# trucndt/oversim

Measured on AMD Instinct MI355X. Metric: routed lookup hops/sec (whole node), higher is better.
Workload: dtype u32 (160-bit keys), int64 ns, fp64 coordinates; 1 GPU; C: Chord 2^20 nodes per GPU (ring sharded over GPUs), 10M random-key iterative one-way lookups per GPU; overlay=chord, nodes_total=1048576, lookups_per_gpu=10000000, hopCountMax=50, parallelism=1 GPU, seed=0xc, successorListSize=8, routingType=iterative

## Files before the change

oversim_amd/csrc/chord.hip:

```cpp
#include <hipcub/hipcub.hpp>

#include "engine.hpp"
#include "launch.hpp"
#include "persist.hpp"

#include <algorithm>
#include <cstdio>
#include <vector>

namespace ovs {


__global__ void k_check_sorted(const KeyRec* __restrict__ recs, uint32_t n, uint32_t* bad)
{
    const uint32_t i = blockIdx.x * blockDim.x + threadIdx.x;
    if (i + 1 < n) {
        const K160 a = key_of(load_rec(recs, i)), b = key_of(load_rec(recs, i + 1));
        if (!k_lt(a, b)) atomicOr(bad, 1u);
    }
}

__global__ void k_chord_rowlen(const KeyRec* __restrict__ recs, uint32_t n, uint32_t lo, uint32_t cnt, uint64_t* rowlen)
{
    const uint32_t t = blockIdx.x * blockDim.x + threadIdx.x;
// ... 35 lines not shown
    FingerEnt* row = fingers + r.aux;
    for (int i = KEYBITS - 1; i >= ilo; --i)
        row[KEYBITS - 1 - i].idx = ring_lower_bound(recs, n, k_add(self, k_pow2(i)));
}

__global__ void k_chord_top(const KeyRec* __restrict__ recs, uint32_t n, int L, FingerEnt* __restrict__ ftop)
{
    const uint64_t t = (uint64_t)blockIdx.x * blockDim.x + threadIdx.x;
    if (t >= (uint64_t)n * (uint32_t)L) return;
    const uint32_t v = (uint32_t)(t / (uint32_t)L);
    const int i = KEYBITS - 1 - (int)(t % (uint32_t)L);
    const K160 self = key_of(load_rec(recs, v));
    ftop[t].idx = ring_lower_bound(recs, n, k_add(self, k_pow2(i)));
}

__global__ void k_chord_nodes(const KeyRec* __restrict__ recs, const double2* __restrict__ xy, uint32_t n, int ns,
                              NodeRec* __restrict__ nodes)
{
    const uint32_t v = blockIdx.x * blockDim.x + threadIdx.x;
    if (v >= n) return;
    const KeyRec r = load_rec(recs, v);
    const K160 C = key_of(r);
    const K160 P = key_of(load_rec(recs, v == 0 ? n - 1 : v - 1));
    const K160 S0 = key_of(load_rec(recs, v + 1 == n ? 0 : v + 1));
    const uint32_t sl = v + (uint32_t)ns >= n ? v + (uint32_t)ns - n : v + (uint32_t)ns;
    const K160 SL = key_of(load_rec(recs, sl));
    const double2 p = xy[v];
    const uint64_t gP = top64(k_sub(P, C)), gS0 = top64(k_sub(S0, C)), gSL = top64(k_sub(SL, C));
    uint4* o = reinterpret_cast<uint4*>(nodes + v);
    o[0] = make_uint4(r.w[0], r.w[1], r.w[2], r.w[3]);
    o[1] = make_uint4(r.w[4], r.aux, (uint32_t)__double2loint(p.x), (uint32_t)__double2hiint(p.x));
    o[2] = make_uint4((uint32_t)__double2loint(p.y), (uint32_t)__double2hiint(p.y), (uint32_t)gS0, (uint32_t)(gS0 >> 32));
    o[3] = make_uint4((uint32_t)gSL, (uint32_t)(gSL >> 32), (uint32_t)gP, (uint32_t)(gP >> 32));
}

__global__ void k_chord_win(const KeyRec* __restrict__ recs, uint32_t n, uint32_t lo, uint32_t cnt, int ns,
                            WinRec* __restrict__ win)
{
    const uint32_t t = blockIdx.x * blockDim.x + threadIdx.x;
    if (t >= cnt) return;
    const uint32_t v = lo + t;
    const K160 C = key_of(load_rec(recs, v));
    uint64_t g[8];
    for (int j = 0; j < 8; ++j) {
        uint32_t sj = v + (uint32_t)j + 1;
        while (sj >= n) sj -= n;
        g[j] = j < ns ? top64(k_sub(key_of(load_rec(recs, sj)), C)) : ~0ull;
    }
    uint4* o = reinterpret_cast<uint4*>(win + t);
    for (int j = 0; j < 4; ++j)
        o[j] = make_uint4((uint32_t)g[2 * j], (uint32_t)(g[2 * j] >> 32), (uint32_t)g[2 * j + 1], (uint32_t)(g[2 * j + 1] >> 32));
}

__global__ void k_chord_entries(const NodeRec* __restrict__ nodes, FingerEnt* __restrict__ ents, uint64_t total)
{
    const uint64_t e = (uint64_t)blockIdx.x * blockDim.x + threadIdx.x;
    if (e >= total) return;
    const uint32_t f = ents[e].idx;
    const uint4* q = reinterpret_cast<const uint4*>(nodes + f);
    const uint4 a = q[0], b = q[1], c = q[2], d = q[3];
    uint4* o = reinterpret_cast<uint4*>(ents + e);
    o[0] = a;
    o[1] = make_uint4(b.x, f, b.z, b.w);
    o[2] = c;
    o[3] = make_uint4(d.x, d.y, b.y, 0u);
}

__global__ void k_chord_export(const KeyRec* __restrict__ recs, const FingerEnt* __restrict__ fingers,
                               uint32_t n, uint32_t* __restrict__ out)
{
    const uint64_t t = (uint64_t)blockIdx.x * blockDim.x + threadIdx.x;
    if (t >= (uint64_t)n * KEYBITS) return;
    const uint32_t v = (uint32_t)(t / KEYBITS);
    const int pos = (int)(t % KEYBITS);
    const KeyRec r = load_rec(recs, v);
    const uint32_t s0i = v + 1 == n ? 0 : v + 1;
    const int ilo = k_msb(k_sub(key_of(load_rec(recs, s0i)), key_of(r))) + 1;
    out[t] = pos >= ilo ? fingers[r.aux + (KEYBITS - 1 - pos)].idx : s0i;
}


struct Decision {
    uint32_t next;
    KeyRec rec;
    uint8_t sib;
    uint8_t broken;
};

__device__ __forceinline__ uint32_t ring_next(uint32_t i, uint32_t d, uint32_t n)
{
    uint32_t j = i + d;
    return j >= n ? j - n : j;
}

__device__ __forceinline__ bool sibling_general(const ChordView& V, uint32_t self, const K160& K,
                                                int numSiblings)
{
    const uint32_t pred = V.pred[self];
    const int ssize = V.nsucc[self];
    const K160 C = key_of(load_rec(V.recs, self));
    if (pred == NONE) {
        const bool isEmpty = ssize == 0 || (ssize == 1 && V.succ[(uint64_t)self * V.sls] == self);
        return isEmpty || k_eq(C, K);
    }
    const K160 PK = key_of(load_rec(V.recs, pred));
    if (between_R(K, PK, C)) return true;
    (void)numSiblings;
    return false;
}

__device__ __forceinline__ Decision decide_general(const ChordView& V, uint32_t c, const KeyRec& crec,
                                                   const K160& K)
{
    Decision d;
    d.broken = 0; d.sib = 0;
    const K160 C = key_of(crec);
    const uint64_t sb = (uint64_t)c * V.sls;
    const int ssize = V.nsucc[c];
// ... 165 lines not shown
    }
}


__device__ __forceinline__ int shard_owner(const uint64_t* __restrict__ lo, int nsh, uint32_t c)
{
    int r = 0;
    for (int i = 1; i < nsh; ++i) r += ((uint64_t)c >= lo[i]) ? 1 : 0;
    return r;
}

__device__ __forceinline__ ovs_lookup_rec load_lrec(const ovs_lookup_rec* __restrict__ p, uint64_t i)
{
    const uint4* q = reinterpret_cast<const uint4*>(p + i);
    const uint4 a = q[0], b = q[1], c = q[2];
    ovs_lookup_rec r;
    r.key[0] = a.x; r.key[1] = a.y; r.key[2] = a.z; r.key[3] = a.w; r.key[4] = b.x;
    r.src = b.y; r.cur = b.z; r.qid = b.w;
    r.t_ns = (int64_t)((uint64_t)c.x | ((uint64_t)c.y << 32));
    r.hops = (uint16_t)(c.z & 0xFFFF);
    r.local = (uint8_t)((c.z >> 16) & 0xFF);
    return r;
}

__device__ __forceinline__ void store_lrec(ovs_lookup_rec* __restrict__ p, uint64_t i, const K160& K, uint32_t S,
                                           uint32_t cur, uint32_t qid, int64_t t, int hops, int local)
{
    uint4* q = reinterpret_cast<uint4*>(p + i);
    q[0] = make_uint4(K.w[0], K.w[1], K.w[2], K.w[3]);
    q[1] = make_uint4(K.w[4], S, cur, qid);
    q[2] = make_uint4((uint32_t)(uint64_t)t, (uint32_t)((uint64_t)t >> 32), (uint32_t)hops | ((uint32_t)local << 16), 0u);
}

enum : uint32_t { PH_FETCH = 0, PH_START = 1, PH_NODE = 2, PH_PROBE = 3, PH_WIN = 4 };

struct Hdr {
    K160 k;
    uint32_t row;
    double x, y;
    uint64_t gS0, gSL;
};

__device__ __forceinline__ void lds_wave_fence()
{
    __builtin_amdgcn_fence(__ATOMIC_RELEASE, "wavefront");
    __builtin_amdgcn_wave_barrier();
    __builtin_amdgcn_fence(__ATOMIC_ACQUIRE, "wavefront");
}

__device__ __forceinline__ int msb64(uint64_t x) { return 63 - __clzll((long long)x); }

__device__ __forceinline__ uint64_t u64(uint32_t lo, uint32_t hi) { return (uint64_t)lo | ((uint64_t)hi << 32); }

__device__ __forceinline__ int cmp_gap(const ChordView& V, const K160& D, uint64_t gt, const K160& C, uint32_t g)
{
    const uint64_t Dt = top64(D);
    if (Dt != gt) return Dt < gt ? -1 : 1;
    const K160 G = k_sub(key_of(load_rec(V.recs, g)), C);
    return k_lt(D, G) ? -1 : (k_eq(D, G) ? 0 : 1);
}

__device__ __forceinline__ uint64_t top64_sub(const K160& a, const K160& b)
{
    const bool borrow = (a.w[2] < b.w[2]) | ((a.w[2] == b.w[2]) & (lo64(a) < lo64(b)));
    return top64(a) - top64(b) - (borrow ? 1u : 0u);
}

struct LaneIO {
    const K160* __restrict__ qkeys;
    const uint32_t* __restrict__ qsrc;
    ovs_route_out* __restrict__ out;
    uint32_t* __restrict__ hopseq;
    const uint32_t* __restrict__ perm;
    const ovs_lookup_rec* __restrict__ in;
    const K160* __restrict__ fkeys;
    const uint32_t* __restrict__ fsrc;
    uint32_t fqid;
    ovs_lookup_rec* __restrict__ sout;
    uint64_t scap;
    unsigned long long* scount;
    ovs_done_rec* __restrict__ done;
    uint64_t dcap;
    unsigned long long* dcount;
    const uint64_t* __restrict__ shard_lo;
    int nsh, me;
    uint64_t n, chunk;
    ovs_lookup_rec* __restrict__ stage_hand;
    ovs_done_rec* __restrict__ stage_done;
    uint8_t* __restrict__ stag;
    unsigned long long* dyn;
    uint64_t dyn_from;
};

constexpr PersistTune K1_TUNE{0.70, 64};

#ifdef OVS_K1_TAIL
__device__ unsigned long long g_k1_tail[2 * PERSIST_TAIL_MAX];
#endif
#ifdef OVS_CHORD_STATS
__device__ unsigned long long g_k1_stats[8];
#endif

#ifndef OVS_K1_WAVES
#define OVS_K1_WAVES 5
#endif
#ifndef OVS_K1_SHARD_WAVES
#define OVS_K1_SHARD_WAVES 5
#endif
template <bool REC, bool RECORD, bool SHARD, bool LKC = false, bool DEF = false>
// ... 312 lines not shown
                cur = nx;
                if (via_node) {
                    nsib = nx_sib; pend = REC;
                    lp = reinterpret_cast<const uint4*>(V.nodes + nx);
                    ph = PH_NODE;
                    return false;
                }
                if (REC) t += DC.msgRoute + coord_ns(sx, sy, A.x, A.y, DC.round);
                asib = nx_sib;
                return true;
            };
            if (!fin && nxt != NONE) arrived = send(nxt, nxt_node, nxt_sib);

            if (arrived) {
                uint32_t nx2 = NONE;
                bool nx2_sib = false;
                const K160 D = k_sub(K, A.k);
                if (ph == PH_START) asib = k_zero(D) || cmp_gap(V, D, u64(L3.z, L3.w), A.k, cur == 0 ? V.n - 1 : cur - 1) > 0;
                if (SHARD && redo) {
                    redo = false;
                    local = false;
                    if (REC) { sx = A.x; sy = A.y; }
                } else if (REC) {
                    const bool at_src = local;
                    local = false;
                    sx = A.x; sy = A.y;
                    if (asib && (!at_src || hops < hcm)) { fin = true; R = cur; }
                    else if (asib || hops >= hcm) { fin = true; status = OVS_LOOKUP_HOPMAX; }
                } else if (local) {
                    local = false;
                    if (asib) { fin = true; R = S; }
                } else {
                    const int64_t cdr = coord_ns(sx, sy, A.x, A.y, DC.round);
                    if (!SHARD) cd = cdr;
                    const int64_t rtt = DC.msgCall + ((LKC && asib) ? DC.msgRespSib : DC.msgResp1) + 2 * cdr;
                    if (rtt >= DC.rpcTimeout) {
                        fin = true;
                        status = (t + DC.rpcTimeout > DC.lookupTimeout) ? OVS_LOOKUP_TIMEOUT : OVS_LOOKUP_RPC_TIMEOUT;
                    } else {
                        t += rtt;
                        if (t > DC.lookupTimeout) { fin = true; status = OVS_LOOKUP_TIMEOUT; }
                        else {
                            if (RECORD && !SHARD && hops < hcm) io.hopseq[dst * (uint64_t)hcm + hops] = cur;
                            ++hops;
                            if (asib) { fin = true; R = cur; }
                        }
                    }
                }
                if (!REC && !fin && hcm && hops >= hcm) { fin = true; status = OVS_LOOKUP_HOPMAX; }
                if (!fin) {
                    C = A.k; row = A.row; gSL = A.gSL; gTx = false;
                    if (!SHARD) Dt = top64(D);
                    const uint32_t s0 = ring_next(cur, 1, V.n);
                    if (cmp_gap(V, D, A.gS0, C, s0) <= 0) {
                        nx2 = s0; nx2_sib = true;
                    } else {
                        ilo = A.gS0 ? 97 + msb64(A.gS0) : k_msb(k_sub(key_of(load_rec(V.recs, s0)), C)) + 1;
                        esl = gSL ? 97 + msb64(gSL) : 96;
                        const uint32_t sl = ring_next(cur, (uint32_t)ns, V.n);
                        const int c = cmp_gap(V, D, gSL, C, sl);
                        if (c < 0) {
                            if (SHARD && remote) {
                                redo_hand();
                            } else {
                                lp = reinterpret_cast<const uint4*>(V.win + (cur - V.lo));
                                ph = PH_WIN;
                            }
                        } else {
                            gTx = c == 0;
                            fb = gTx ? ring_next(cur, (uint32_t)ns - 1, V.n) : sl;
                            pi = k_msb(D);
                            if (pi >= ilo) {
                                if (SHARD && remote && pi < KEYBITS - V.ftl) {
                                    redo_hand();
                                } else {
                                    lp = fptr(pi);
                                    ph = PH_PROBE;
                                }
                            } else {
                                nx2 = fb;
                            }
                        }
                    }
                }
                if (!fin && nx2 != NONE) send(nx2, true, nx2_sib);
            }

            if (fin) {
                ovs_route_out o;
                if (REC) {
                    const bool ok = status == OVS_LOOKUP_OK;
                    o.hops = (uint16_t)(ok ? hops : 0);
                    o.one_way_hops = (uint8_t)(ok ? hops : 0);
                    o.latency_ns = ok ? t : -1;
                    o.responsible = ok ? R : NONE;
                } else if (status == OVS_LOOKUP_OK) {
                    o.hops = (uint16_t)hops;
                    o.responsible = R;
                    o.one_way_hops = (uint8_t)(hops + (R != S ? 1 : 0));
                    o.latency_ns = t + ((R != S && !LKC) ? DC.msgRoute + (SHARD ? coord_ns(sx, sy, A.x, A.y, DC.round) : cd) : 0);
                } else {
                    o.hops = (uint16_t)hops;
                    o.responsible = NONE;
                    o.one_way_hops = 0;
                    o.latency_ns = -1;
                }
                o.status = status;
                if (SHARD) {
                    ovs_done_rec dr;
                    dr.qid = qid; dr.pad = 0; dr.out = o;
                    io.stage_done[q] = dr;
                    io.stag[q] = (uint8_t)io.nsh;
                } else {
                    static_assert(sizeof(ovs_route_out) == 16 && alignof(ovs_route_out) == 8, "one 16 B record");
                    reinterpret_cast<uint4*>(io.out)[dst] =
                        make_uint4(o.responsible, (uint32_t)o.hops | ((uint32_t)o.status << 16) | ((uint32_t)o.one_way_hops << 24),
                                   (uint32_t)(uint64_t)o.latency_ns, (uint32_t)((uint64_t)o.latency_ns >> 32));
// ... 103 lines not shown
    out[i] = 2 * bw + DC.access2 + coord_ns(p.x, p.y, r.x, r.y, DC.round);
}


hipError_t launch_check_sorted(const KeyRec* recs, uint32_t n, uint32_t* bad, hipStream_t s)
{
    if (n < 2) return hipSuccess;
    hipLaunchKernelGGL(k_check_sorted, dim3(nblk(n, 256)), dim3(256), 0, s, recs, n, bad);
    return hipGetLastError();
}

hipError_t launch_chord_build(KeyRec* recs, uint32_t n, uint32_t lo, uint32_t hi, FingerEnt** fingers_out,
                              uint64_t* nfing_out, hipStream_t s)
{
    hipError_t e;
    uint64_t* rowlen = nullptr;
    uint64_t* off = nullptr;
    void* tmp = nullptr;
    size_t tmpb = 0;
    const uint32_t cnt = hi - lo;
    *fingers_out = nullptr;
    if ((e = hipMalloc(&rowlen, sizeof(uint64_t) * (cnt + 1))) != hipSuccess) return e;
    if ((e = hipMalloc(&off, sizeof(uint64_t) * (cnt + 1))) != hipSuccess) { hipFree(rowlen); return e; }
    hipLaunchKernelGGL(k_chord_rowlen, dim3(nblk(cnt, 256)), dim3(256), 0, s, recs, n, lo, cnt, rowlen);
    hipMemsetAsync(rowlen + cnt, 0, sizeof(uint64_t), s);
    hipcub::DeviceScan::ExclusiveSum(nullptr, tmpb, rowlen, off, cnt + 1, s);
    if ((e = hipMalloc(&tmp, tmpb)) != hipSuccess) { hipFree(rowlen); hipFree(off); return e; }
    hipcub::DeviceScan::ExclusiveSum(tmp, tmpb, rowlen, off, cnt + 1, s);
    uint64_t total = 0;
    hipMemcpyAsync(&total, off + cnt, sizeof(uint64_t), hipMemcpyDeviceToHost, s);
    hipStreamSynchronize(s);
    if (total + KEYBITS >= 0xFFFFFFFFull) { hipFree(rowlen); hipFree(off); hipFree(tmp); return hipErrorInvalidValue; }
    FingerEnt* fing = nullptr;
    if ((e = hipMalloc(&fing, sizeof(FingerEnt) * (total + KEYBITS))) != hipSuccess) {
        hipFree(rowlen); hipFree(off); hipFree(tmp); return e;
    }
    hipMemsetAsync(fing, 0, sizeof(FingerEnt) * (total + KEYBITS), s);
    hipLaunchKernelGGL(k_set_aux, dim3(nblk(cnt, 256)), dim3(256), 0, s, recs, off, lo, cnt);
    hipLaunchKernelGGL(k_chord_fill, dim3(nblk(cnt, 128)), dim3(128), 0, s, recs, n, lo, cnt, fing);
    e = hipStreamSynchronize(s);
    hipFree(rowlen); hipFree(off); hipFree(tmp);
    if (e != hipSuccess) { hipFree(fing); return e; }
    *fingers_out = fing;
    *nfing_out = total;
    return hipGetLastError();
}

hipError_t launch_chord_nodes(const KeyRec* recs, const double2* xy, uint32_t n, int ns, NodeRec* nodes,
                              FingerEnt* fingers, uint64_t nfing, WinRec* win, uint32_t lo, uint32_t hi, hipStream_t s)
{
    if (n == 0) return hipSuccess;
    hipLaunchKernelGGL(k_chord_nodes, dim3(nblk(n, 256)), dim3(256), 0, s, recs, xy, n, ns, nodes);
    if (hi > lo) hipLaunchKernelGGL(k_chord_win, dim3(nblk(hi - lo, 256)), dim3(256), 0, s, recs, n, lo, hi - lo, ns, win);
    if (nfing) hipLaunchKernelGGL(k_chord_entries, dim3(nblk(nfing, 256)), dim3(256), 0, s, nodes, fingers, nfing);
    return hipGetLastError();
}

hipError_t launch_chord_top(const KeyRec* recs, uint32_t n, int L, FingerEnt* ftop, hipStream_t s)
{
    const uint64_t tot = (uint64_t)n * (uint32_t)L;
    if (tot == 0) return hipSuccess;
    hipLaunchKernelGGL(k_chord_top, dim3(nblk(tot, 256)), dim3(256), 0, s, recs, n, L, ftop);
    return hipGetLastError();
}

hipError_t launch_chord_entries(const NodeRec* nodes, FingerEnt* ents, uint64_t total, hipStream_t s)
{
    if (total == 0) return hipSuccess;
    hipLaunchKernelGGL(k_chord_entries, dim3(nblk(total, 256)), dim3(256), 0, s, nodes, ents, total);
    return hipGetLastError();
}

hipError_t launch_chord_export(const KeyRec* recs, const FingerEnt* fingers, uint32_t n, uint32_t* out,
                               hipStream_t s)
{
    const uint64_t tot = (uint64_t)n * KEYBITS;
    hipLaunchKernelGGL(k_chord_export, dim3(nblk(tot, 256)), dim3(256), 0, s, recs, fingers, n, out);
    return hipGetLastError();
}

template <bool REC, bool RECORD, bool SHARD, bool LKC = false, bool DEF = false>
static hipError_t lanes_launch(const ChordView& V, const DelayConsts& DC, const LookupConsts& LC, LaneIO io,
                               int num_cu, hipStream_t s)
{
    const PersistPlan pl = persist_plan(io.n, persist_waves<k_chord_lanes<REC, RECORD, SHARD, LKC, DEF>>(num_cu),
                                        io.dyn != nullptr, K1_TUNE);
    const uint64_t blocks = pl.blocks;
    io.chunk = pl.chunk;
    io.dyn_from = pl.dyn_from;
    if (!pl.dyn) io.dyn = nullptr;
#ifdef OVS_CHORD_STATS
    unsigned long long z[8] = {};
    hipMemcpyToSymbolAsync(HIP_SYMBOL(g_k1_stats), z, sizeof z, 0, hipMemcpyHostToDevice, s);
#endif
    hipLaunchKernelGGL((k_chord_lanes<REC, RECORD, SHARD, LKC, DEF>), dim3((unsigned)blocks), dim3(256), 0, s, V, DC,
                       LC, io);
#ifdef OVS_K1_TAIL
    if (!SHARD) persist_tail_report("k1tail", HIP_SYMBOL(g_k1_tail), blocks * 4, io.chunk, s);
#endif
#ifdef OVS_CHORD_STATS
    hipMemcpyFromSymbolAsync(z, HIP_SYMBOL(g_k1_stats), sizeof z, 0, hipMemcpyDeviceToHost, s);
    hipStreamSynchronize(s);
    fprintf(stderr, "k1stats n=%llu fetch=%llu start=%llu node=%llu probe1=%llu reprobe=%llu win=%llu "
            "wave_iters=%llu busy_lanes=%llu\n",
            (unsigned long long)io.n, z[0], z[1], z[2], z[3], z[4], z[5], z[6], z[7]);
#endif
    return hipGetLastError();
}

template <bool IDEAL, bool RECORD, bool REC>
static hipError_t chord_route_launch(const ChordView& V, const DelayConsts& DC, const LookupConsts& LC,
                                     const K160* qkeys, const uint32_t* qsrc, uint64_t nq, ovs_route_out* out,
                                     uint32_t* hopseq, int num_cu, hipStream_t s, const uint32_t* perm = nullptr,
                                     unsigned long long* dyn = nullptr)
{
    if constexpr (IDEAL) {
        LaneIO io{};
        io.qkeys = qkeys; io.qsrc = qsrc; io.out = out; io.hopseq = hopseq; io.n = nq; io.perm = perm;
        io.dyn = dyn;
        if constexpr (!REC && !RECORD) {
            if (DC.lookupCall) return lanes_launch<false, false, false, true>(V, DC, LC, io, num_cu, s);
        }
// ... 270 lines not shown
```

oversim_amd/csrc/engine.hpp:

```cpp
#pragma once
#include <hip/hip_runtime.h>
#include <stdint.h>

#include "key160.hpp"
#include "../../include/ovs_kbr.h"

namespace ovs {

constexpr uint32_t NONE = 0xFFFFFFFFu;
constexpr int KEYBITS = 160;

inline uint64_t up256(uint64_t b) { return (b + 255) & ~255ull; }

inline unsigned nblk(uint64_t n, unsigned b) { return (unsigned)((n + b - 1) / b); }

struct DelayConsts {
    int64_t msgCall;
    int64_t msgResp1;
    int64_t msgRoute;
    int64_t rpcTimeout;
    int64_t lookupTimeout;
    int32_t round;
    int32_t respBase;
    int32_t respPerNode;
    int32_t callBytes;
    int32_t routeBytes;
    double datarate;
    int64_t access2;
    int64_t msgRespSib;
    int32_t lookupCall;
    int64_t bwCall;
    int64_t bwRoute;
    int64_t bwResp[17];
};


__device__ __forceinline__ int64_t simtime_ns(double seconds, int round)
{
    const double x = __dmul_rn(seconds, 1e9);
    return round ? (int64_t)floor(__dadd_rn(x, 0.5)) : (int64_t)x;
}

__device__ __forceinline__ int64_t coord_ns(double ax, double ay, double bx, double by, int round)
{
    const double dx = __dsub_rn(ax, bx);
    const double dy = __dsub_rn(ay, by);
    const double s = __dadd_rn(__dmul_rn(dx, dx), __dmul_rn(dy, dy));
    const float f = __double2float_rn(__dsqrt_rn(s));
    return simtime_ns(__dmul_rn(0.001, (double)f), round);
}

__device__ __forceinline__ int64_t bw_ns(int32_t bytes, double datarate, int round)
{
    return simtime_ns(__ddiv_rn((double)((int64_t)bytes * 8), datarate), round);
// ... 1 lines not shown

__device__ __forceinline__ int64_t resp_ns(const DelayConsts& DC, int nodes)
{
    return 2 * bw_ns(DC.respBase + DC.respPerNode * nodes, DC.datarate, DC.round) + DC.access2;
}

__device__ __forceinline__ KeyRec load_rec(const KeyRec* __restrict__ recs, uint32_t i)
{
    const uint2* p = reinterpret_cast<const uint2*>(recs + i);
    const uint2 a = p[0], b = p[1], c = p[2];
    KeyRec r;
    r.w[0] = a.x; r.w[1] = a.y; r.w[2] = b.x; r.w[3] = b.y; r.w[4] = c.x; r.aux = c.y;
    return r;
}

__device__ __forceinline__ K160 rkey(const KeyRec* __restrict__ recs, uint64_t i) { return key_of(load_rec(recs + i, 0)); }

__device__ __forceinline__ uint64_t vis_bit(uint32_t x) { return 1ull << ((x * 0x9E3779B1u) >> 26); }

__device__ __forceinline__ ovs_route_out iter_route_out(uint8_t status, int hops, int64_t t, uint32_t responsible, uint32_t S,
                                                        double sx, double sy, double rx, double ry, const DelayConsts& DC)
{
    ovs_route_out o;
    o.hops = (uint16_t)hops;
    o.status = status;
    if (status == OVS_LOOKUP_OK) {
        o.responsible = responsible;
        o.one_way_hops = (uint8_t)(hops + (responsible != S ? 1 : 0));
        int64_t lat = t;
        if (responsible != S) lat += DC.msgRoute + coord_ns(sx, sy, rx, ry, DC.round);
        o.latency_ns = lat;
    } else {
        o.responsible = NONE;
        o.one_way_hops = 0;
        o.latency_ns = -1;
    }
    return o;
}

struct alignas(64) NodeRec {
    uint32_t w[5];
    uint32_t row;
    double x, y;
    uint64_t gS0;
    uint64_t gSL;
    uint64_t gP;
};
static_assert(sizeof(NodeRec) == 64, "NodeRec is one 64 B line");

struct alignas(64) FingerEnt {
    uint32_t w[5];
    uint32_t idx;
    double x, y;
    uint64_t gS0;
    uint64_t gSL;
    uint32_t row;
    uint32_t pad;
};
static_assert(sizeof(FingerEnt) == 64, "FingerEnt is one 64 B line");

struct alignas(64) WinRec {
    uint64_t g[8];
};

__device__ __host__ __forceinline__ uint64_t top64(const K160& a) { return (uint64_t)a.w[3] | ((uint64_t)a.w[4] << 32); }

__device__ __forceinline__ double dbl(uint32_t lo, uint32_t hi) { return __hiloint2double((int)hi, (int)lo); }

struct ChordView {
    const KeyRec* __restrict__ recs;
    const double2* __restrict__ xy;
    const NodeRec* __restrict__ nodes;
    const FingerEnt* __restrict__ frow;
    const WinRec* __restrict__ win;
    uint32_t lo;
    const uint32_t* __restrict__ pred;
    const uint32_t* __restrict__ succ;
    const uint8_t* __restrict__ nsucc;
    const uint32_t* __restrict__ fres;
    uint32_t n;
    int32_t ns;
    int32_t sls;
    int32_t numFingerCandidates;
    const FingerEnt* __restrict__ ftop;
    int32_t ftl;
};

constexpr int MAXSHARDS = 64;
struct ShardMap {
    uint64_t lo[MAXSHARDS + 1];
    int n;
};

struct LookupConsts {
    int32_t hopCountMax;
    int32_t numSiblings;
    int32_t numRedundantNodes;
    int32_t recursive;
};

}
```

oversim_amd/csrc/launch.hpp:

```cpp
#pragma once
#include "engine.hpp"
#include "compact.hpp"

namespace ovs {

hipError_t launch_check_sorted(const KeyRec* recs, uint32_t n, uint32_t* bad, hipStream_t s);
hipError_t launch_chord_build(KeyRec* recs, uint32_t n, uint32_t lo, uint32_t hi, FingerEnt** fingers_out,
                              uint64_t* nfing_out, hipStream_t s);
hipError_t launch_chord_shard_step(const ChordView& V, const DelayConsts& DC, const LookupConsts& LC,
                                   const uint64_t* shard_lo, int nsh, int me, const ovs_lookup_rec* in, uint64_t nin,
                                   ovs_lookup_rec* out, uint64_t out_cap,
                                   unsigned long long* out_count, ovs_done_rec* done, uint64_t done_cap,
                                   unsigned long long* done_count, StageBuf& stage, int num_cu, hipStream_t s,
                                   const K160* fkeys = nullptr, const uint32_t* fsrc = nullptr, uint32_t fqid = 0,
                                   unsigned long long* dyn = nullptr);
hipError_t launch_make_records(const KeyRec* recs, const K160* keys, const uint32_t* src, uint64_t n, uint32_t qid_base,
                               ovs_lookup_rec* out, hipStream_t s);
hipError_t launch_chord_nodes(const KeyRec* recs, const double2* xy, uint32_t n, int ns, NodeRec* nodes,
                              FingerEnt* fingers, uint64_t nfing, WinRec* win, uint32_t lo, uint32_t hi, hipStream_t s);
hipError_t launch_chord_top(const KeyRec* recs, uint32_t n, int L, FingerEnt* ftop, hipStream_t s);
hipError_t launch_chord_entries(const NodeRec* nodes, FingerEnt* ents, uint64_t total, hipStream_t s);
hipError_t launch_chord_export(const KeyRec* recs, const FingerEnt* fingers, uint32_t n, uint32_t* out,
                               hipStream_t s);
hipError_t launch_chord_route(const ChordView& V, bool ideal, const DelayConsts& DC, const LookupConsts& LC,
                              const K160* qkeys, const uint32_t* qsrc, uint64_t nq, ovs_route_out* out,
                              uint32_t* hopseq, int num_cu, hipStream_t s, const uint32_t* perm = nullptr,
                              unsigned long long* dyn = nullptr);
uint64_t ksort_scratch_words();
hipError_t ksort_launch(const K160* keys, const uint32_t* src, uint64_t n, uint32_t* scratch, K160* skeys,
                        uint32_t* ssrc, uint32_t* perm, int bits, hipStream_t s);
hipError_t launch_chord_find_node(const ChordView& V, bool ideal, const uint32_t* node, const K160* keys,
                                  uint64_t n, int numRedundant, int numSiblings, uint32_t* out_nodes,
                                  uint32_t max_out, uint8_t* out_count, uint8_t* out_sib, hipStream_t s);
hipError_t launch_shard_lookup_finish(const ChordView& V, int ns, const ovs_done_rec* done, ovs_lookup_out* out,
                                      uint32_t* sibs, uint64_t n, hipStream_t s);
hipError_t launch_chord_exact_finish(const ChordView& V, const DelayConsts& DC, int hcm, const K160* keys,
                                     const uint32_t* src, const uint32_t* hopseq, int H, ovs_route_out* io,
                                     uint64_t n, hipStream_t s);
hipError_t launch_lookup_finish(const ChordView& V, bool chord, bool ideal, int ns, ovs_route_out* io,
                                uint32_t* sibs, uint64_t n, hipStream_t s);
hipError_t launch_fill_rpcs_from_hops(const ovs_route_out* out, uint64_t n, uint32_t* rpcs, hipStream_t s);
hipError_t launch_xy_bbox(const double2* xy, uint64_t n, double* out, int* blocks, hipStream_t s);
hipError_t launch_delay(const double2* xy, const DelayConsts& DC, const uint32_t* a, const uint32_t* b,
                        const int32_t* bytes, uint64_t n, int64_t* out, hipStream_t s);

}
```

oversim_amd/csrc/ovs_load.cpp:

```cpp
#include <algorithm>
#include <string>
#include <type_traits>
#include <vector>

#include "ctx.hpp"

using namespace ovs;

namespace ovs {

ChordView chord_view(const ovs_ctx* c)
{
    ChordView V{};
    V.recs = c->recs; V.xy = c->xy; V.nodes = c->nodes; V.frow = c->fingers; V.win = c->win;
    V.lo = (uint32_t)c->shard_lo;
    V.pred = c->pred; V.succ = c->succ;
    V.nsucc = c->nsucc; V.fres = c->fres; V.n = (uint32_t)c->n;
    V.ns = (int)std::min<uint64_t>((uint64_t)c->P.successorListSize, c->n - 1);
    V.sls = c->sls;
    V.numFingerCandidates = c->P.numFingerCandidates;
    V.ftop = c->ftop; V.ftl = c->ftop ? c->ftl : 0;
    return V;
}

ovs_status ensure_nodes(ovs_ctx* c, hipStream_t s)
{
    if (!c->ideal || c->overlay != OVS_OVERLAY_CHORD) return OVS_OK;
    const int ns = (int)std::min<uint64_t>((uint64_t)c->P.successorListSize, c->n - 1);
    if (c->nodes && c->nodes_ns == ns) return OVS_OK;
    if (ns < 1) return fail(c, OVS_EINVAL, "successorListSize must be >= 1");
    if (!c->nodes) HIPCHK(c, hipMalloc(&c->nodes, sizeof(NodeRec) * c->n));
    if (!c->win) HIPCHK(c, hipMalloc(&c->win, sizeof(WinRec) * (c->shard_hi - c->shard_lo)));
    HIPCHK(c, launch_chord_nodes(c->recs, c->xy, (uint32_t)c->n, ns, c->nodes, c->fingers, c->nfing, c->win,
                                 (uint32_t)c->shard_lo, (uint32_t)c->shard_hi, s));
    if (c->ftop) HIPCHK(c, launch_chord_entries(c->nodes, c->ftop, c->n * (uint64_t)c->ftl, s));
    HIPCHK(c, hipStreamSynchronize(s));
    c->nodes_ns = ns;
    return OVS_OK;
}

ovs_status upload_nodes(ovs_ctx* c, const ovs_key160* ids, uint64_t n, const double* xy, bool dev)
{
    if (n < 2) return fail(c, OVS_EINVAL, "need at least 2 nodes");
    if (n >= 0xFFFFFFFFull) return fail(c, OVS_EINVAL, "too many nodes for 32-bit node indices");
    if (dev) HIPCHK(c, hipDeviceSynchronize());
    HIPCHK(c, hipMalloc(&c->recs, sizeof(KeyRec) * n));
    HIPCHK(c, hipMalloc(&c->xy, sizeof(double2) * n));
    HIPCHK(c, hipMemset2DAsync(c->recs, sizeof(KeyRec), 0, sizeof(KeyRec), n, c->stream));
    HIPCHK(c, hipMemcpy2DAsync(c->recs, sizeof(KeyRec), ids, sizeof(ovs_key160), sizeof(ovs_key160), n,
                               dev ? hipMemcpyDeviceToDevice : hipMemcpyHostToDevice, c->stream));
    HIPCHK(c, hipMemcpyAsync(c->xy, xy, sizeof(double2) * n, dev ? hipMemcpyDeviceToDevice : hipMemcpyHostToDevice,
                             c->stream));
    CallFrame F(false, c->stream);
    uint32_t hbad = 0;
    uint32_t* bad = F.out(&hbad, 1);
    if (!F.ok()) return frame_fail(c, F);
    HIPCHK(c, hipMemsetAsync(bad, 0, sizeof(uint32_t), c->stream));
    HIPCHK(c, launch_check_sorted(c->recs, (uint32_t)n, bad, c->stream));
    if (F.finish() != hipSuccess) return frame_fail(c, F);
    if (hbad) return fail(c, OVS_EINVAL, "node ids must be sorted ascending and unique");
    c->n = n;
    return OVS_OK;
}

static ovs_status upload_finger_rows(ovs_ctx* c, const uint32_t* rows, uint64_t m)
{
    const uint64_t n = c->n;
    if (m * 8 >= n) {
        HIPCHK(c, hipMemcpy(c->fres, c->ch.fres.data(), sizeof(uint32_t) * n * 160, hipMemcpyHostToDevice));
        return OVS_OK;
    }
    for (uint64_t j = 0; j < m; ++j)
        HIPCHK(c, hipMemcpy(c->fres + (uint64_t)rows[j] * 160, c->ch.fres.data() + (uint64_t)rows[j] * 160,
                            sizeof(uint32_t) * 160, hipMemcpyHostToDevice));
    return OVS_OK;
}

hipError_t kad_build_from_host(ovs_ctx* c, const uint32_t* siblings, const uint8_t* bucket_count,
                               const uint32_t* bucket_nodes, KadTables& T, bool* staged, uint32_t bad[2])
{
    const uint64_t n = c->n, S5 = 5ull * (uint64_t)c->P.s, k = (uint64_t)c->P.k;
    CallFrame F(false, c->stream);
    uint32_t* dsib = F.scratch<uint32_t>(n * S5);
    uint8_t* dbc = F.scratch<uint8_t>(n * 160);
    uint32_t* dbn = F.scratch<uint32_t>(n * 160 * k);
    if (!(*staged = F.ok())) return F.error();
    hipError_t e = hipMemcpy(dsib, siblings, sizeof(uint32_t) * n * S5, hipMemcpyHostToDevice);
    if (e == hipSuccess) e = hipMemcpy(dbc, bucket_count, n * 160, hipMemcpyHostToDevice);
// ... 382 lines not shown
```

oversim_amd/csrc/ovs_shard.cpp:

```cpp
#include <algorithm>
#include <string>

#include "ctx.hpp"

using namespace ovs;

namespace ovs {
namespace {

ovs_status upload_bounds(ovs_ctx* c, const uint64_t* lo, uint32_t nshards)
{
    if (!c->d_bounds) HIPCHK(c, hipMalloc(&c->d_bounds, sizeof(uint64_t) * (MAXSHARDS + 1)));
    if (c->h_bounds.size() == nshards + 1 && std::equal(lo, lo + nshards + 1, c->h_bounds.begin())) return OVS_OK;
    HIPCHK(c, hipDeviceSynchronize());
    HIPCHK(c, hipMemcpy(c->d_bounds, lo, sizeof(uint64_t) * (nshards + 1), hipMemcpyHostToDevice));
    c->h_bounds.assign(lo, lo + nshards + 1);
    return OVS_OK;
}

ovs_status arc_map(ovs_ctx* c, const uint64_t* shard_lo, uint32_t nshards, uint64_t lo, uint64_t hi, int* me)
{
    uint64_t bounds[MAXSHARDS + 1];
    std::string err;
    if (ovs_status st = check_arc_map(shard_lo, nshards, c->n, lo, hi, bounds, me, &err)) return fail(c, st, err);
// ... 82 lines not shown

ovs_status kad_shard_reset_errors(ovs_ctx* c, void* stream)
{
    HIPCHK(c, hipSetDevice(c->device));
    if (!c->kbad) HIPCHK(c, hipMalloc(&c->kbad, sizeof(unsigned long long)));
    HIPCHK(c, hipMemsetAsync(c->kbad, 0, sizeof(unsigned long long), (hipStream_t)stream));
    return OVS_OK;
}

ovs_status kad_mig_step_impl(ovs_ctx* c, const void* in, uint64_t n_in, const ovs_key160* fkeys, const uint32_t* fsrc,
                             uint32_t fqid, void* out, uint64_t out_cap, unsigned long long* out_count, ovs_done_rec* done,
                             uint64_t done_cap, unsigned long long* done_count, const uint64_t* shard_lo,
                             uint32_t nshards, void* stream, bool reset_errors)
{
    if (!c || !shard_lo || nshards == 0 || nshards > (uint32_t)MAXSHARDS) return OVS_EINVAL;
    if (n_in && ((!in && !(fkeys && fsrc)) || !out || !out_count || !done || !done_count)) return OVS_EINVAL;
    if (c->overlay != OVS_OVERLAY_KADEMLIA) return fail(c, OVS_ESTATE, "no Kademlia network loaded");
    ovs_status st = check_common(c, c->P);
    if (st != OVS_OK) return st;
    if (!kad_mig_supported(c->P, c->kad))
        return fail(c, OVS_ENOTSUP, "the migration step implements one-way iterative KBR routes on snapshot tables with "
                                    "k and lookupRedundantNodes <= 8");
    int me = -1;
    if ((st = arc_map(c, shard_lo, nshards, c->kad.lo, c->kad.hi, &me)) != OVS_OK) return st;
    hipStream_t s = (hipStream_t)stream;
    if (!c->kbad || reset_errors)
        if ((st = kad_shard_reset_errors(c, stream)) != OVS_OK) return st;
    const DynSlots::Lease dyn = dyn_acquire(c, n_in, s);
    hipError_t e = kad_mig_step(c->kad, c->xy, (uint32_t)c->n, c->P, delay_consts(c->P), in, n_in,
                                reinterpret_cast<const K160*>(fkeys), fsrc, fqid, c->d_bounds, (int)nshards, me, out,
                                out_cap, out_count, done, done_cap, done_count, c->kbad, c->num_cu, c->stage[s], s,
                                dyn.get());
    return e == hipSuccess ? OVS_OK : hip_fail(c, e, "kademlia migration step");
}

}

extern "C" {

ovs_status ovs_chord_shard_replicate(ovs_ctx* c, int32_t top_levels)
{
    if (!c) return OVS_EINVAL;
    if (c->overlay != OVS_OVERLAY_CHORD || !c->ideal) return fail(c, OVS_ESTATE, "no Chord ring (shard) loaded");
    if (top_levels < 0 || top_levels > 32) return fail(c, OVS_EINVAL, "top_levels must be 0..32");
    HIPCHK(c, hipSetDevice(c->device));
    HIPCHK(c, hipDeviceSynchronize());
    if (c->ftop) hipFree(c->ftop);
    c->ftop = nullptr; c->ftl = 0;
    if (top_levels == 0) return OVS_OK;
    const uint64_t tot = c->n * (uint64_t)top_levels;
    HIPCHK(c, hipMalloc(&c->ftop, sizeof(FingerEnt) * tot));
    c->ftl = top_levels;
    HIPCHK(c, launch_chord_top(c->recs, (uint32_t)c->n, top_levels, c->ftop, c->stream));
    if (c->nodes) HIPCHK(c, launch_chord_entries(c->nodes, c->ftop, tot, c->stream));
    HIPCHK(c, hipStreamSynchronize(c->stream));
    return OVS_OK;
}

int32_t ovs_chord_shard_levels(const ovs_ctx* c) { return c && c->ftop ? c->ftl : 0; }

ovs_status ovs_shard_make_records(ovs_ctx* c, const ovs_key160* keys, const uint32_t* src, uint64_t n,
                                  uint32_t qid_base, ovs_lookup_rec* recs, void* stream)
{
    if (!c || (n && (!keys || !src || !recs))) return OVS_EINVAL;
    if (c->overlay != OVS_OVERLAY_CHORD || !c->ideal) return fail(c, OVS_ESTATE, "no Chord ring (shard) loaded");
    HIPCHK(c, hipSetDevice(c->device));
    hipStream_t s = (hipStream_t)stream;
    HIPCHK(c, launch_make_records(c->recs, reinterpret_cast<const K160*>(keys), src, n, qid_base, recs, s));
    return OVS_OK;
}

ovs_status ovs_shard_step_keys(ovs_ctx* c, int32_t num_siblings, const ovs_key160* keys, const uint32_t* src, uint64_t n,
                               uint32_t qid_base, ovs_lookup_rec* out, uint64_t out_cap, unsigned long long* out_count,
                               ovs_done_rec* done, uint64_t done_cap, unsigned long long* done_count,
                               const uint64_t* shard_lo, uint32_t nshards, void* stream)
{
    if (!c || (n && (!keys || !src))) return OVS_EINVAL;
    int32_t ns = 0;
    if (num_siblings != 0)
        if (ovs_status st = shard_lookup_ns(c, num_siblings, true, &ns)) return st;
    return shard_step(c, ns, nullptr, n, out, out_cap, out_count, done, done_cap, done_count, shard_lo, nshards, stream,
                      keys, src, qid_base);
}

ovs_status ovs_shard_step(ovs_ctx* c, const ovs_lookup_rec* in, uint64_t n_in, ovs_lookup_rec* out, uint64_t out_cap,
                          unsigned long long* out_count, ovs_done_rec* done, uint64_t done_cap,
                          unsigned long long* done_count, const uint64_t* shard_lo, uint32_t nshards, void* stream)
{
    return shard_step(c, 0, in, n_in, out, out_cap, out_count, done, done_cap, done_count, shard_lo, nshards, stream);
}

ovs_status ovs_shard_step_lookup(ovs_ctx* c, int32_t num_siblings, const ovs_lookup_rec* in, uint64_t n_in,
                                 ovs_lookup_rec* out, uint64_t out_cap, unsigned long long* out_count,
                                 ovs_done_rec* done, uint64_t done_cap, unsigned long long* done_count,
                                 const uint64_t* shard_lo, uint32_t nshards, void* stream)
{
    if (!c) return OVS_EINVAL;
    int32_t ns = 0;
    if (ovs_status st = shard_lookup_ns(c, num_siblings, true, &ns)) return st;
    return shard_step(c, ns, in, n_in, out, out_cap, out_count, done, done_cap, done_count, shard_lo, nshards, stream);
}

ovs_status ovs_shard_lookup_finish(ovs_ctx* c, const ovs_done_rec* done, uint64_t n, int32_t num_siblings,
                                   ovs_lookup_out* out, uint32_t* siblings, void* stream)
{
    if (!c || (n && (!done || !out || !siblings))) return OVS_EINVAL;
    if (c->overlay != OVS_OVERLAY_CHORD || !c->ideal) return fail(c, OVS_ESTATE, "no Chord ring (shard) loaded");
// ... 136 lines not shown
```

Measured before the change: 41.03 billion hops/s.

## Embed 8-bit successor-window codes in finger entries to skip window fetch

Finger entries now carry 8-bit quantized gaps to the successors 2 through 7, packed into the low 16 bits of gS0 and the former pad word, with gS0 truncated by 16 bits. When routing lands in the successor window, the kernel scans these codes and picks the next hop directly, which avoids loading the 64-byte window record unless two codes tie. In exchange the gS0 comparison loses precision, and finger-entry setup has to do extra ring key loads. The fast path only fires when ph==PH_PROBE and the table was built with successorListSize 8.

```diff
diff --git a/oversim_amd/csrc/chord.hip b/oversim_amd/csrc/chord.hip
--- a/oversim_amd/csrc/chord.hip
+++ b/oversim_amd/csrc/chord.hip
@@ -111,18 +111,34 @@
         o[j] = make_uint4((uint32_t)g[2 * j], (uint32_t)(g[2 * j] >> 32), (uint32_t)g[2 * j + 1], (uint32_t)(g[2 * j + 1] >> 32));
 }
 
-__global__ void k_chord_entries(const NodeRec* __restrict__ nodes, FingerEnt* __restrict__ ents, uint64_t total)
+__global__ void k_chord_entries(const KeyRec* __restrict__ recs, uint32_t n, int ns, const NodeRec* __restrict__ nodes,
+                                FingerEnt* __restrict__ ents, uint64_t total)
 {
     const uint64_t e = (uint64_t)blockIdx.x * blockDim.x + threadIdx.x;
     if (e >= total) return;
     const uint32_t f = ents[e].idx;
     const uint4* q = reinterpret_cast<const uint4*>(nodes + f);
     const uint4 a = q[0], b = q[1], c = q[2], d = q[3];
+    const uint64_t gS0 = (uint64_t)c.z | ((uint64_t)c.w << 32), gSL = (uint64_t)d.x | ((uint64_t)d.y << 32);
+    uint64_t g[6] = {};
+    if (ns == 8 && gSL) {
+        K160 C;
+        C.w[0] = a.x; C.w[1] = a.y; C.w[2] = a.z; C.w[3] = a.w; C.w[4] = b.x;
+        #pragma unroll
+        for (int j = 1; j <= 6; ++j) {
+            uint32_t sj = f + (uint32_t)j + 1;
+            while (sj >= n) sj -= n;
+            g[j - 1] = top64(k_sub(key_of(load_rec(recs, sj)), C));
+        }
+    }
+    uint64_t gS0c;
+    uint32_t wc;
+    finger_pack(gS0, gSL, g, ns == 8, &gS0c, &wc);
     uint4* o = reinterpret_cast<uint4*>(ents + e);
     o[0] = a;
     o[1] = make_uint4(b.x, f, b.z, b.w);
-    o[2] = c;
-    o[3] = make_uint4(d.x, d.y, b.y, 0u);
+    o[2] = make_uint4(c.x, c.y, (uint32_t)gS0c, (uint32_t)(gS0c >> 32));
+    o[3] = make_uint4(d.x, d.y, b.y, wc);
 }
 
 __global__ void k_chord_export(const KeyRec* __restrict__ recs, const FingerEnt* __restrict__ fingers,
@@ -394,9 +410,11 @@
 
 __device__ __forceinline__ uint64_t u64(uint32_t lo, uint32_t hi) { return (uint64_t)lo | ((uint64_t)hi << 32); }
 
+template <int DROP = 0>
 __device__ __forceinline__ int cmp_gap(const ChordView& V, const K160& D, uint64_t gt, const K160& C, uint32_t g)
 {
-    const uint64_t Dt = top64(D);
+    const uint64_t Dt = top64(D) >> DROP;
+    gt >>= DROP;
     if (Dt != gt) return Dt < gt ? -1 : 1;
     const K160 G = k_sub(key_of(load_rec(V.recs, g)), C);
     return k_lt(D, G) ? -1 : (k_eq(D, G) ? 0 : 1);
@@ -815,17 +833,26 @@
                     C = A.k; row = A.row; gSL = A.gSL; gTx = false;
                     if (!SHARD) Dt = top64(D);
                     const uint32_t s0 = ring_next(cur, 1, V.n);
-                    if (cmp_gap(V, D, A.gS0, C, s0) <= 0) {
+                    if (cmp_gap<FINGER_GS0_DROP>(V, D, A.gS0, C, s0) <= 0) {
                         nx2 = s0; nx2_sib = true;
                     } else {
-                        ilo = A.gS0 ? 97 + msb64(A.gS0) : k_msb(k_sub(key_of(load_rec(V.recs, s0)), C)) + 1;
+                        ilo = (A.gS0 >> FINGER_GS0_DROP) ? 97 + msb64(A.gS0) : k_msb(k_sub(key_of(load_rec(V.recs, s0)), C)) + 1;
                         esl = gSL ? 97 + msb64(gSL) : 96;
                         const uint32_t sl = ring_next(cur, (uint32_t)ns, V.n);
                         const int c = cmp_gap(V, D, gSL, C, sl);
                         if (c < 0) {
+                            bool coded = false;
+                            if (!SHARD && ph == PH_PROBE) {
+                                const uint64_t codes = finger_codes(A.gS0, L3.w);
+                                if (finger_has_codes(codes)) {
+                                    bool tie;
+                                    const int tj = finger_win_scan(codes, (uint32_t)(top64(D) >> max(esl - 104, 0)), &tie);
+                                    if (!tie) { nx2 = ring_next(cur, (uint32_t)tj + 1, V.n); coded = true; }
+                                }
+                            }
                             if (SHARD && remote) {
                                 redo_hand();
-                            } else {
+                            } else if (!coded) {
                                 lp = reinterpret_cast<const uint4*>(V.win + (cur - V.lo));
                                 ph = PH_WIN;
                             }
@@ -1035,7 +1062,7 @@
     if (n == 0) return hipSuccess;
     hipLaunchKernelGGL(k_chord_nodes, dim3(nblk(n, 256)), dim3(256), 0, s, recs, xy, n, ns, nodes);
     if (hi > lo) hipLaunchKernelGGL(k_chord_win, dim3(nblk(hi - lo, 256)), dim3(256), 0, s, recs, n, lo, hi - lo, ns, win);
-    if (nfing) hipLaunchKernelGGL(k_chord_entries, dim3(nblk(nfing, 256)), dim3(256), 0, s, nodes, fingers, nfing);
+    if (nfing) hipLaunchKernelGGL(k_chord_entries, dim3(nblk(nfing, 256)), dim3(256), 0, s, recs, n, ns, nodes, fingers, nfing);
     return hipGetLastError();
 }
 
@@ -1047,10 +1074,11 @@
     return hipGetLastError();
 }
 
-hipError_t launch_chord_entries(const NodeRec* nodes, FingerEnt* ents, uint64_t total, hipStream_t s)
+hipError_t launch_chord_entries(const KeyRec* recs, uint32_t n, int ns, const NodeRec* nodes, FingerEnt* ents,
+                                uint64_t total, hipStream_t s)
 {
     if (total == 0) return hipSuccess;
-    hipLaunchKernelGGL(k_chord_entries, dim3(nblk(total, 256)), dim3(256), 0, s, nodes, ents, total);
+    hipLaunchKernelGGL(k_chord_entries, dim3(nblk(total, 256)), dim3(256), 0, s, recs, n, ns, nodes, ents, total);
     return hipGetLastError();
 }
 
diff --git a/oversim_amd/csrc/engine.hpp b/oversim_amd/csrc/engine.hpp
--- a/oversim_amd/csrc/engine.hpp
+++ b/oversim_amd/csrc/engine.hpp
@@ -1,5 +1,6 @@
 #pragma once
 #include <hip/hip_runtime.h>
+#include <stddef.h>
 #include <stdint.h>
 
 #include "key160.hpp"
@@ -107,18 +108,69 @@
     uint32_t w[5];
     uint32_t idx;
     double x, y;
-    uint64_t gS0;
+    uint64_t gS0c;
     uint64_t gSL;
     uint32_t row;
-    uint32_t pad;
+    uint32_t wc;
 };
 static_assert(sizeof(FingerEnt) == 64, "FingerEnt is one 64 B line");
+static_assert(offsetof(FingerEnt, gS0c) == offsetof(NodeRec, gS0) && offsetof(FingerEnt, gSL) == offsetof(NodeRec, gSL),
+              "a lane unpacks either line the same way");
 
 struct alignas(64) WinRec {
     uint64_t g[8];
 };
 
 __device__ __host__ __forceinline__ uint64_t top64(const K160& a) { return (uint64_t)a.w[3] | ((uint64_t)a.w[4] << 32); }
+
+constexpr int FINGER_GS0_DROP = 16;
+constexpr uint64_t FINGER_NO_CODES = 0x0000000000FFull;
+
+__device__ __host__ __forceinline__ int finger_code_shift(uint64_t gSL)
+{
+    const int m = gSL ? 63 - __builtin_clzll(gSL) : 0;
+    return m > 7 ? m - 7 : 0;
+}
+
+__device__ __host__ __forceinline__ uint64_t finger_codes(uint64_t gS0c, uint32_t wc)
+{
+    return (gS0c & 0xFFFFull) | ((uint64_t)wc << 16);
+}
+
+__device__ __host__ __forceinline__ bool finger_has_codes(uint64_t codes)
+{
+    return (uint32_t)(codes & 0xFF) <= (uint32_t)(codes >> 40);
+}
+
+__device__ __host__ __forceinline__ uint64_t finger_gs0(uint64_t gS0c) { return gS0c & ~0xFFFFull; }
+
+__device__ __host__ __forceinline__ void finger_pack(uint64_t gS0, uint64_t gSL, const uint64_t (&g)[6], bool coded,
+                                                     uint64_t* gS0c, uint32_t* wc)
+{
+    uint64_t codes = FINGER_NO_CODES;
+    if (coded && gSL) {
+        const int sh = finger_code_shift(gSL);
+        codes = 0;
+#pragma unroll
+        for (int j = 0; j < 6; ++j) codes |= ((g[j] >> sh) & 0xFF) << (8 * j);
+    }
+    *gS0c = finger_gs0(gS0) | (codes & 0xFFFF);
+    *wc = (uint32_t)(codes >> 16);
+}
+
+__device__ __host__ __forceinline__ int finger_win_scan(uint64_t codes, uint32_t cD, bool* tie)
+{
+    int tj = 0;
+    bool eq = false;
+#pragma unroll
+    for (int j = 0; j < 6; ++j) {
+        const uint32_t cj = (uint32_t)(codes >> (8 * j)) & 0xFF;
+        tj += cj < cD ? 1 : 0;
+        eq |= cj == cD;
+    }
+    *tie = eq;
+    return tj;
+}
 
 __device__ __forceinline__ double dbl(uint32_t lo, uint32_t hi) { return __hiloint2double((int)hi, (int)lo); }
 
diff --git a/oversim_amd/csrc/launch.hpp b/oversim_amd/csrc/launch.hpp
--- a/oversim_amd/csrc/launch.hpp
+++ b/oversim_amd/csrc/launch.hpp
@@ -19,7 +19,8 @@
 hipError_t launch_chord_nodes(const KeyRec* recs, const double2* xy, uint32_t n, int ns, NodeRec* nodes,
                               FingerEnt* fingers, uint64_t nfing, WinRec* win, uint32_t lo, uint32_t hi, hipStream_t s);
 hipError_t launch_chord_top(const KeyRec* recs, uint32_t n, int L, FingerEnt* ftop, hipStream_t s);
-hipError_t launch_chord_entries(const NodeRec* nodes, FingerEnt* ents, uint64_t total, hipStream_t s);
+hipError_t launch_chord_entries(const KeyRec* recs, uint32_t n, int ns, const NodeRec* nodes, FingerEnt* ents,
+                                uint64_t total, hipStream_t s);
 hipError_t launch_chord_export(const KeyRec* recs, const FingerEnt* fingers, uint32_t n, uint32_t* out,
                                hipStream_t s);
 hipError_t launch_chord_route(const ChordView& V, bool ideal, const DelayConsts& DC, const LookupConsts& LC,
diff --git a/oversim_amd/csrc/ovs_load.cpp b/oversim_amd/csrc/ovs_load.cpp
--- a/oversim_amd/csrc/ovs_load.cpp
+++ b/oversim_amd/csrc/ovs_load.cpp
@@ -33,7 +33,7 @@
     if (!c->win) HIPCHK(c, hipMalloc(&c->win, sizeof(WinRec) * (c->shard_hi - c->shard_lo)));
     HIPCHK(c, launch_chord_nodes(c->recs, c->xy, (uint32_t)c->n, ns, c->nodes, c->fingers, c->nfing, c->win,
                                  (uint32_t)c->shard_lo, (uint32_t)c->shard_hi, s));
-    if (c->ftop) HIPCHK(c, launch_chord_entries(c->nodes, c->ftop, c->n * (uint64_t)c->ftl, s));
+    if (c->ftop) HIPCHK(c, launch_chord_entries(c->recs, (uint32_t)c->n, ns, c->nodes, c->ftop, c->n * (uint64_t)c->ftl, s));
     HIPCHK(c, hipStreamSynchronize(s));
     c->nodes_ns = ns;
     return OVS_OK;
diff --git a/oversim_amd/csrc/ovs_shard.cpp b/oversim_amd/csrc/ovs_shard.cpp
--- a/oversim_amd/csrc/ovs_shard.cpp
+++ b/oversim_amd/csrc/ovs_shard.cpp
@@ -158,7 +158,7 @@
     HIPCHK(c, hipMalloc(&c->ftop, sizeof(FingerEnt) * tot));
     c->ftl = top_levels;
     HIPCHK(c, launch_chord_top(c->recs, (uint32_t)c->n, top_levels, c->ftop, c->stream));
-    if (c->nodes) HIPCHK(c, launch_chord_entries(c->nodes, c->ftop, tot, c->stream));
+    if (c->nodes) HIPCHK(c, launch_chord_entries(c->recs, (uint32_t)c->n, c->nodes_ns, c->nodes, c->ftop, tot, c->stream));
     HIPCHK(c, hipStreamSynchronize(c->stream));
     return OVS_OK;
 }
```

Measured after the change: 42.75 billion hops/s (median of 6 runs). +4.2%, better.
